# ScanNet/ScanNet

Measured on AMD Instinct MI355X. Metric: RGB-D frames/sec integrated (640x480, 4 mm voxel), higher is better.
Workload: dtype f32; 1 GPU; configs[1]: scene0000_00-scale synthetic stream (5578-frame box-room walk, 640x480 u16 depth, 4 mm voxels, 2^19 hash buckets x 10, 2^20 SDF blocks), frames 5..24 per rank, depth AND colour (a 640x480 RGB8 frame per depth frame, 921 600 B) resident in HBM; frames_per_pass=32, blocks_live_end=34141, alloc_failures=0

## Files before the change

include/scanfuse_internal.h:

```cpp
#ifndef SCANFUSE_INTERNAL_H
#define SCANFUSE_INTERNAL_H

#include "scanfuse.h"

#ifdef __cplusplus
extern "C" {
#endif

int sf_fuser_tune(sf_fuser* f, const char* key, int value);

int sf_fuser_alloc_probe_count(sf_fuser* f, uint64_t* out);

int sf_fuser_alloc_direct_count(sf_fuser* f, uint64_t* out);

int sf_fuser_mc_timing(const sf_fuser* f, double* out, int n);

int sf_zlib_inflate_gpu(const void* src, uint64_t src_bytes, uint64_t expect_bytes, int device, void* dst);
int sf_zlib_inflate_gpu_bench(const void* const* srcs, const uint64_t* src_bytes, int count, uint64_t expect_bytes, int device, int repeats, int skip, double* us_tokens, double* us_copy);

int sf_fuse_run_device_counts(uint64_t out[4]);

int sf_jpeg_decode_gpu_huffman(const uint8_t* data, uint64_t bytes, uint32_t width, uint32_t height, int device, uint8_t* dst_rgb);

int sf_fuser_profile_enable(sf_fuser* f, int on);
// ... 53 lines not shown
```

scannet_amd/csrc/fuser.hip:

```cpp
#include <hip/hip_runtime.h>

#include <algorithm>
#include <climits>
#include <cmath>
#include <cstdlib>
#include <cstring>
#include <string>
#include <vector>

#include "fuser_internal.h"

hipError_t sf_quiesce(sf_fuser* f) {
  hipError_t e = hipSuccess;
  if (f->front) e = hipStreamSynchronize(f->front);
  if (f->front_lo) { const hipError_t e1 = hipStreamSynchronize(f->front_lo); if (e == hipSuccess) e = e1; }
  const hipError_t e2 = hipStreamSynchronize(f->stream);
  return e != hipSuccess ? e : e2;
}

namespace {

bool frame_setup(const sf_params& p, const float* pose, FrameK& f) {
  if (pose[0] == -INFINITY) return false;
  for (int i = 0; i < 12; i++) f.T[i] = pose[i];
// ... 67 lines not shown
  hipStream_t sa = sf_input_stream(f, n, col, sign);
  if (f->overlap && sa != s) {
    if (f->last_front != nullptr && f->last_front != sa) {
      (void)hipEventRecord(f->ev_front_switch, f->last_front);
      (void)hipStreamWaitEvent(sa, f->ev_front_switch, 0);
    }
    f->last_front = sa;
    if (f->serial_tail) {
      (void)hipEventRecord(f->ev_input, s);
      (void)hipStreamWaitEvent(sa, f->ev_input, 0);
      f->serial_tail = false;
    }
    (void)hipStreamWaitEvent(sa, f->ev_fused[sl], 0);
  }
  const bool fuse_pre = f->alloc_ray && n == 1 && sign > 0 && !col && f->pk.inW == 0 && !rs;
  if (!fuse_pre) sf_launch_prepass(f, sl, rs ? n_planes : n, in, sa);
  if (sign > 0) sf_launch_alloc(f, sl, n, bf, in, sa, fuse_pre);
  sf_launch_compact(f, sl, bf, sa);
  if (f->overlap && sa != s) {
    (void)hipEventRecord(f->ev_compact[sl], sa);
    (void)hipStreamWaitEvent(s, f->ev_compact[sl], 0);
  }
  hipEvent_t e0 = nullptr, e1 = nullptr;
  if (f->profile) {
    if (f->events_used == f->events.size()) {
      hipEvent_t a, b;
      if (hipEventCreate(&a) != hipSuccess || hipEventCreate(&b) != hipSuccess) return sf::fail(SF_ERR_DEVICE, "hipEventCreate failed");
      f->events.emplace_back(a, b);
    }
    e0 = f->events[f->events_used].first;
    e1 = f->events[f->events_used].second;
    f->events_used++;
    (void)hipEventRecord(e0, s);
  }
  if (rs) sf_launch_reintegrate(f, sl, col, bt, *rs, s);
  else sf_launch_integrate(f, sl, n, sign, col, bt, s);
  if (f->profile) (void)hipEventRecord(e1, s);
  if (f->overlap && sa != s) (void)hipEventRecord(f->ev_fused[sl], s);
  if (f->overlap && sa == s) f->serial_tail = true;
  f->pipe_beside = f->pipe_overlap == 1 || (f->pipe_overlap < 0 && sf_big_pass(f));
  if ((f->pipe_beside || f->front_prio == 0) && f->front_lo == nullptr && f->overlap) {
    int prio_lo = 0, prio_hi = 0;
    hipError_t e_ = hipSuccess;
    if (f->front_lo_lowest) {
      e_ = hipDeviceGetStreamPriorityRange(&prio_lo, &prio_hi);
      if (e_ == hipSuccess) e_ = hipStreamCreateWithPriority(&f->front_lo, hipStreamNonBlocking, prio_lo);
    } else {
      e_ = hipStreamCreateWithFlags(&f->front_lo, hipStreamNonBlocking);
    }
    if (e_ != hipSuccess) {
// ... 106 lines not shown
    hipError_t e_ = hipMalloc((void**)&(ptr), (bytes));                                           \
    if (e_ != hipSuccess) {                                                                       \
      sf_fuser_destroy(f);                                                                        \
      return sf::fail(SF_ERR_DEVICE, "hipMalloc(%zu bytes) failed: %s", (size_t)(bytes), hipGetErrorString(e_)); \
    }                                                                                             \
  } while (0)
  SF_CREATE_CHECK(hipStreamCreateWithFlags(&f->stream, hipStreamNonBlocking));
  {
    int prio_lo = 0, prio_hi = 0;
    SF_CREATE_CHECK(hipDeviceGetStreamPriorityRange(&prio_lo, &prio_hi));
    SF_CREATE_CHECK(hipStreamCreateWithPriority(&f->front, hipStreamNonBlocking, prio_hi));
    SF_CREATE_CHECK(hipEventCreateWithFlags(&f->ev_front_switch, hipEventDisableTiming));
  }
  for (int q = 0; q < 2; q++) {
    SF_CREATE_CHECK(hipEventCreateWithFlags(&f->ev_compact[q], hipEventDisableTiming));
    SF_CREATE_CHECK(hipEventCreateWithFlags(&f->ev_fused[q], hipEventDisableTiming));
  }
  SF_CREATE_CHECK(hipEventCreateWithFlags(&f->ev_input, hipEventDisableTiming));
  SF_ALLOC(f->table, (size_t)k.total_slots * sizeof(HashEntry));
  {
    uint32_t lines = 1024;
    while ((uint64_t)lines * 64ull < (uint64_t)k.num_blocks && lines < (1u << 24)) lines <<= 1;
    f->brick_lines = lines;
    SF_ALLOC(f->bricks, (size_t)lines * 8 * 16);
  }
  SF_ALLOC(f->heap, (size_t)k.num_blocks * 4);
  SF_ALLOC(f->block_keys, (size_t)k.num_blocks * 8);
  SF_ALLOC(f->block_entry, (size_t)k.num_blocks * 4);
  SF_ALLOC(f->block_flags, (size_t)k.num_blocks);
  SF_ALLOC(f->voxels, (size_t)k.num_blocks * 4096);
// ... 34 lines not shown
#undef SF_CREATE_CHECK
  *out = f;
  return SF_OK;
}

SF_API void sf_fuser_destroy(sf_fuser* f) {
  if (!f) return;
  (void)hipSetDevice(f->device);
  if (f->front) (void)hipStreamSynchronize(f->front);
  if (f->front_lo) (void)hipStreamSynchronize(f->front_lo);
  if (f->stream) (void)hipStreamSynchronize(f->stream);
  for (auto& e : f->events) { (void)hipEventDestroy(e.first); (void)hipEventDestroy(e.second); }
  (void)hipFree(f->table); (void)hipFree(f->bricks); (void)hipFree(f->heap); (void)hipFree(f->block_keys); (void)hipFree(f->block_entry); (void)hipFree(f->block_flags); (void)hipFree(f->voxels);
  for (int q = 0; q < 2; q++) { (void)hipFree(f->depthf2[q]); (void)hipFree(f->color2[q]); (void)hipFree(f->compact2[q]); (void)hipFree(f->cmask2[q]); }
  (void)hipFree(f->counters); (void)hipFree(f->ray_kx); (void)hipFree(f->ray_ky); (void)hipFree(f->void_depth);
  for (int q = 0; q < 2; q++) { if (f->ev_compact[q]) (void)hipEventDestroy(f->ev_compact[q]); if (f->ev_fused[q]) (void)hipEventDestroy(f->ev_fused[q]); }
  if (f->ev_input) (void)hipEventDestroy(f->ev_input);
  if (f->front) { (void)hipStreamSynchronize(f->front); (void)hipStreamDestroy(f->front); }
  if (f->front_lo) { (void)hipStreamSynchronize(f->front_lo); (void)hipStreamDestroy(f->front_lo); }
  if (f->ev_front_switch) (void)hipEventDestroy(f->ev_front_switch);
  for (hipEvent_t e : f->ev_raycast) if (e) (void)hipEventDestroy(e);
  sf_track_release(f);
  sf_align_release(f);
  for (int q = 0; q < sf_fuser::HOST_RING; q++) {
    (void)hipFree(f->staging_depth[q]); (void)hipFree(f->staging_rgb[q]);
    if (f->pinned_depth[q]) (void)hipHostFree(f->pinned_depth[q]);
    if (f->pinned_rgb[q]) (void)hipHostFree(f->pinned_rgb[q]);
    if (f->ev_h2d[q]) (void)hipEventDestroy(f->ev_h2d[q]);
    if (f->ev_consumed[q]) (void)hipEventDestroy(f->ev_consumed[q]);
  }
  if (f->host_mirror) (void)hipHostFree(f->host_mirror);
// ... 70 lines not shown
  return fuse_host(f, depth, rgb, pose, +1);
}
SF_API int sf_fuser_deintegrate(sf_fuser* f, const uint16_t* depth, const uint8_t* rgb, const float pose[16]) {
  return fuse_host(f, depth, rgb, pose, -1);
}
SF_API int sf_fuser_integrate_device(sf_fuser* f, const void* d_depth, const void* d_rgb, const float pose[16]) {
  if (!f || !d_depth || !pose) return sf::fail(SF_ERR_INVALID_ARG, "NULL argument");
  SF_HIP_CHECK(hipSetDevice(f->device));
  return run_frame(f, d_depth, d_rgb, pose, +1);
}
SF_API int sf_fuser_deintegrate_device(sf_fuser* f, const void* d_depth, const void* d_rgb, const float pose[16]) {
  if (!f || !d_depth || !pose) return sf::fail(SF_ERR_INVALID_ARG, "NULL argument");
  SF_HIP_CHECK(hipSetDevice(f->device));
  return run_frame(f, d_depth, d_rgb, pose, -1);
}
static int integrate_batch_device(sf_fuser* f, const void* d_depth, uint64_t frame_stride_bytes, const void* d_rgb, uint64_t rgb_stride_bytes, const float* poses,
                                  uint64_t n) {
  if (!f || !d_depth || !poses) return sf::fail(SF_ERR_INVALID_ARG, "NULL argument");
  SF_HIP_CHECK(hipSetDevice(f->device));
  const void* dd[MAX_BATCH];
  const void* dr[MAX_BATCH];
  const float* pp[MAX_BATCH];
  int m = 0;
  int pass = 0;
  for (uint64_t i = 0; i <= n; i++) {
    if (i < n) {
      if (poses[16 * i] == -INFINITY) { f->frames_skipped++; continue; }
      dd[m] = (const uint8_t*)d_depth + i * frame_stride_bytes;
      dr[m] = d_rgb ? (const uint8_t*)d_rgb + i * rgb_stride_bytes : nullptr;
      pp[m] = poses + 16 * i;
      m++;
    }
    constexpr int ramp = 8;
    int want = f->batch;
    if (ramp < f->batch && n > (uint64_t)ramp) {
      if (n <= (uint64_t)f->batch) want = (int)((n + 1) / 2);
      else if (pass == 0) want = ramp;
      else if (pass < 6) want = std::min(f->batch, ramp << pass);
    }
    if (m == want || (i == n && m > 0)) {
      f->tail_pass = i == n;
      f->head_pass = pass == 0 && n > (uint64_t)m;
      const int rc = run_batch(f, dd, d_rgb ? dr : nullptr, pp, m, +1);
      f->tail_pass = false;
      f->head_pass = false;
      if (rc != SF_OK) return rc;
      m = 0;
      pass++;
    }
  }
  return SF_OK;
}
SF_API int sf_fuser_integrate_batch_device(sf_fuser* f, const void* d_depth, uint64_t frame_stride_bytes, const float* poses, uint64_t n) {
  return integrate_batch_device(f, d_depth, frame_stride_bytes, nullptr, 0, poses, n);
}
SF_API int sf_fuser_integrate_batch_device_rgb(sf_fuser* f, const void* d_depth, uint64_t frame_stride_bytes, const void* d_rgb, uint64_t rgb_stride_bytes,
                                               const float* poses, uint64_t n) {
  if (!d_rgb) return sf::fail(SF_ERR_INVALID_ARG, "NULL colour frames (sf_fuser_integrate_batch_device is the geometry-only entry point)");
  return integrate_batch_device(f, d_depth, frame_stride_bytes, d_rgb, rgb_stride_bytes, poses, n);
}
// ... 122 lines not shown
  if (!f || !key) return sf::fail(SF_ERR_INVALID_ARG, "NULL argument");
  SF_HIP_CHECK(hipSetDevice(f->device));
  SF_HIP_CHECK(sf_quiesce(f));
  const std::string k(key);
  auto in = [&](int lo, int hi) { return value >= lo && value <= hi; };
  if (k == "batch" && in(1, MAX_BATCH)) f->batch = value;
  else if (k == "overlap" && in(0, 1)) f->overlap = value != 0;
  else if (k == "xcd_walk" && in(0, 1)) f->xcd_walk = value != 0;
  else if (k == "pipe" && in(0, 1)) f->pipe_mode = value;
  else if (k == "pipe_overlap" && in(-1, 1)) { f->pipe_overlap = value; f->pipe_beside = value == 1; }
  else if (k == "alloc_group" && in(1, MAX_BATCH)) f->alloc_group = value;
  else if (k == "front_prio" && in(-1, 1)) f->front_prio = value;
  else if (k == "front_lo_lowest" && in(0, 1)) f->front_lo_lowest = value != 0;
  else if (k == "alloc_ray" && in(0, 1)) f->alloc_ray = value != 0;
  else if (k == "tail_wide" && in(0, 1)) f->tail_wide = value;
  else if (k == "brick_cache" && in(0, 1)) {
    f->brick_on = value != 0;
    SF_HIP_CHECK(hipMemsetAsync(f->bricks, 0, (size_t)f->brick_lines * 128, f->stream));
    SF_HIP_CHECK(sf_quiesce(f));
  }
  else return sf::fail(SF_ERR_INVALID_ARG, "sf_fuser_tune: unknown key or value out of range: %s = %d", key, value);
  return SF_OK;
}

int sf_fuser_run_batch(sf_fuser* f, const void* const* d_depth, const void* const* d_rgb, const float* const* poses, int n) {
  if (n < 1 || n > f->batch) return sf::fail(SF_ERR_INVALID_ARG, "batch of %d frames (limit %d)", n, f->batch);
  return run_batch(f, d_depth, d_rgb, poses, n, +1);
}

int sf_fuser_run_batch_ycc(sf_fuser* f, const void* const* d_depth, const void* const* d_planes, const void* const* d_layout, const float* const* poses, int n) {
// ... 92 lines not shown
```

scannet_amd/csrc/fuser_alloc.hip:

```cpp
#include <hip/hip_runtime.h>

#include <algorithm>
#include <climits>
#include <cmath>

#include "fuser_device.h"
#include "fuser_internal.h"

namespace {

__device__ inline int world_to_block(float w, float voxel, float rv) {
  const float q = div_rn(w, voxel, rv);
  const int vi = (int)(q >= 0.0f ? q + 0.5f : q - 0.5f);
  return vi >> 3;
}

constexpr int ALLOC_SET = 256;
constexpr int ALLOC_LIST = 512;
constexpr int ALLOC_SET_PROBES = 32;

template <int WIN_LOG2, bool MULTI>
__global__ __launch_bounds__(256) void k_alloc(const float* __restrict__ depthf_all, HashEntry* table, int32_t* heap,
                                               uint64_t* block_keys, int32_t* block_entry, uint8_t* block_flags, int32_t* counters, ParamsK P,
                                               BatchFrames B, int group_frames, BrickCache bricks) {
// ... 692 lines not shown
  hipLaunchKernelGGL((k_alloc_ray<MULTI>), grid, dim3(256), 0, s, f->depthf2[sl], f->table, f->heap, f->block_keys, f->block_entry, f->block_flags,
                     f->counters, f->pk, bf, gf, raw_depth, f->depthf2[sl], sf_compact_counter(sl));
}

}

void sf_alloc_choose_window(sf_fuser* f, const sf_params* p) {
  const float seg = 2.0f * (p->trunc_base + p->trunc_scale * p->max_integration_dist) / (8.0f * p->voxel_size);
  f->alloc_win64 = seg > 20.0f;
  const float bsz = 8.0f * p->voxel_size;
  const float half_tile = 8.0f * p->max_integration_dist / std::min(p->fx, p->fy);
  const float reach = (p->max_integration_dist + p->trunc_base + p->trunc_scale * p->max_integration_dist) * 1.25f;
  f->alloc_ray = half_tile / bsz <= 4.0f && reach / bsz <= (float)(RW_DEPTH - 6);
}

void sf_launch_alloc(const sf_fuser* f, int sl, int n, const BatchFrames& bf, const BatchIn& in, hipStream_t s, bool fuse_pre) {
  const int group = f->head_pass ? std::min(f->alloc_group, 4) : f->alloc_group;
  const bool win64 = f->alloc_win64 && !f->alloc_ray;
  const int gf = win64 ? 1 : std::min(group, n);
  const dim3 ag((f->p.depth_width + 15) / 16, (f->p.depth_height + 15) / 16, (n + gf - 1) / gf);
  if (f->alloc_ray) {
    const uint16_t* raw_depth = fuse_pre ? in.depth[0] : nullptr;
    if (gf == 1) launch_alloc_ray<false>(f, sl, ag, bf, gf, raw_depth, s);
    else launch_alloc_ray<true>(f, sl, ag, bf, gf, raw_depth, s);
  }
  else if (win64) launch_alloc<6, false>(f, sl, ag, bf, gf, s);
  else if (gf == 1) launch_alloc<5, false>(f, sl, ag, bf, gf, s);
  else launch_alloc<5, true>(f, sl, ag, bf, gf, s);
}
```

scannet_amd/csrc/fuser_compact.hip:

```cpp
#include <hip/hip_runtime.h>

#include <cstring>

#include "fuser_device.h"
#include "fuser_internal.h"

namespace {

constexpr int COMPACT_FEW = 4;

struct CompactArgs {
  const uint64_t* block_keys;
  const int32_t* block_entry;
  const uint8_t* block_flags;
  const HashEntry* table;
  int32_t* compact;
  uint32_t* cmask;
  int32_t* counters;
  int counter_id, all_live;
  ParamsK P;
  BatchFrames B;
};
constexpr int FRAMEK_WORDS = (int)(sizeof(FrameK) / 4);

constexpr int COMPACT_THREADS = 256;
constexpr int COMPACT_WAVES = COMPACT_THREADS / 64;

__global__ __launch_bounds__(COMPACT_THREADS) void k_compactify(CompactArgs A) {
  const uint64_t* __restrict__ block_keys = A.block_keys;
  const int32_t* __restrict__ block_entry = A.block_entry;
  const uint8_t* __restrict__ block_flags = A.block_flags;
  const HashEntry* __restrict__ table = A.table;
  int32_t* __restrict__ compact = A.compact;
  uint32_t* __restrict__ cmask = A.cmask;
// ... 17 lines not shown
    typedef __attribute__((address_space(4))) const uint32_t* karg_t;
    typedef __attribute__((address_space(4))) const char* kbyte_t;
    const karg_t kp = (karg_t)((kbyte_t)__builtin_amdgcn_kernarg_segment_ptr() + offsetof(CompactArgs, B) + offsetof(BatchFrames, f));
    for (int i = threadIdx.x; i < B.n * FRAMEK_WORDS; i += COMPACT_THREADS) s_fk[i] = kp[i];
    __syncthreads();
    uint32_t* fw = reinterpret_cast<uint32_t*>(&F);
    const uint32_t* mine = s_fk + (q < B.n ? q : 0) * FRAMEK_WORDS;
#pragma unroll
    for (int i = 0; i < FRAMEK_WORDS; i++) fw[i] = mine[i];
  }
  for (int base = blockIdx.x * COMPACT_THREADS; base < hw; base += gridDim.x * COMPACT_THREADS) {
    const int i = base + (int)threadIdx.x;
    uint32_t m = 0u;
    if (wide) {
      int4 c = make_int4(0, 0, 0, 0);
      if (i < hw) {
        const uint64_t k = block_keys[i];
        if (k != KEY_EMPTY && !(block_flags[i] & 1)) {
          unpack_key(k, c.x, c.y, c.z);
          c.w = 1;
        }
      }
      s_c[threadIdx.x] = c;
      __syncthreads();
      const uint64_t gmask = fshift == 5 ? 0xFFFFFFFFull : ((1ull << (1 << fshift)) - 1ull);
#pragma unroll 2
      for (int e0 = wave * 64; e0 < wave * 64 + 64; e0 += epi) {
        const int4 cc = s_c[e0 + sub];
        const bool in = cc.w != 0 && q < B.n && block_in_frustum(P, F, cc.x, cc.y, cc.z);
        const uint64_t bal = __ballot(in);
        if (q == 0) s_m[e0 + sub] = (uint32_t)((bal >> (sub << fshift)) & gmask);
      }
      __syncthreads();
      m = s_m[threadIdx.x];
      if (m != 0u) {
        const uint32_t birth = table[block_entry[i]].birth;
        if (birth > B.seq0) {
          const uint32_t d = birth - B.seq0;
          m = d >= 32u ? 0u : (m & ~((1u << d) - 1u));
        }
      }
    }
    const uint64_t bal = __ballot(m != 0u);
    const int rank = __popcll((unsigned long long)(bal & ((1ull << lane) - 1ull)));
    const int wtotal = __popcll((unsigned long long)bal);
    const int wlast = __popcll((unsigned long long)__ballot((m & last_bit) != 0u));
    int pop = __popc(m);
    for (int o = 32; o > 0; o >>= 1) pop += __shfl_xor(pop, o);
    if (lane == 0) { s_wtot[wave] = wtotal; s_wlast[wave] = wlast; s_wpop[wave] = pop; }
    __syncthreads();
    if (threadIdx.x == 0) {
      int total = 0, tlast = 0;
      for (int w = 0; w < COMPACT_WAVES; w++) { total += s_wtot[w]; tlast += s_wlast[w]; }
      s_base = 0;
      if (total) {
        const unsigned long long add = (unsigned long long)(uint32_t)total | ((unsigned long long)(uint32_t)tlast << 32);
        s_base = (int)(uint32_t)atomicAdd(reinterpret_cast<unsigned long long*>(&counters[counter_id]), add);
      }
    } else if (threadIdx.x == 64 && !all_live) {
      int total = 0, tpop = 0;
      for (int w = 0; w < COMPACT_WAVES; w++) { total += s_wtot[w]; tpop += s_wpop[w]; }
      if (total) {
        atomicAdd(reinterpret_cast<unsigned long long*>(&counters[C_TOTAL_LO]), (unsigned long long)tpop);
        atomicAdd(reinterpret_cast<unsigned long long*>(&counters[C_TILES_LO]), (unsigned long long)total);
      }
    }
    __syncthreads();
    int off = s_base;
    for (int w = 0; w < wave; w++) off += s_wtot[w];
    if (m != 0u) {
      compact[off + rank] = i;
      cmask[off + rank] = m;
    }
    __syncthreads();
  }
}

__global__ __launch_bounds__(COMPACT_THREADS) void k_compactify_few(CompactArgs A) {
  const uint64_t* __restrict__ block_keys = A.block_keys;
  const int32_t* __restrict__ block_entry = A.block_entry;
// ... 20 lines not shown
#pragma unroll
    for (int u = 0; u < EU; u++) {
      const int i = base + u * COMPACT_THREADS + (int)threadIdx.x;
      k[u] = i < hw ? block_keys[i] : KEY_EMPTY;
      fl[u] = i < hw ? block_flags[i] : (uint8_t)0;
    }
    int wlast = 0, pop = 0;
#pragma unroll
    for (int u = 0; u < EU; u++) {
      m[u] = 0u;
      if (k[u] != KEY_EMPTY && !(all_live != 1 && (fl[u] & 1))) {
        if (all_live) m[u] = 1u;
        else {
          int bx, by, bz;
          unpack_key(k[u], bx, by, bz);
          for (int qq = 0; qq < B.n; qq++)
            if (block_in_frustum(P, B.f[qq], bx, by, bz)) m[u] |= 1u << qq;
          if (m[u] != 0u && B.n > 1) {
            const uint32_t birth = table[block_entry[base + u * COMPACT_THREADS + (int)threadIdx.x]].birth;
            if (birth > B.seq0) {
              const uint32_t d = birth - B.seq0;
              m[u] = d >= 32u ? 0u : (m[u] & ~((1u << d) - 1u));
            }
          }
        }
      }
      const uint64_t bal = __ballot(m[u] != 0u);
      rank[u] = __popcll((unsigned long long)(bal & ((1ull << lane) - 1ull)));
      if (lane == 0) s_ut[u][wave] = __popcll((unsigned long long)bal);
      wlast += __popcll((unsigned long long)__ballot((m[u] & last_bit) != 0u));
      pop += __popc(m[u]);
    }
    for (int o = 32; o > 0; o >>= 1) pop += __shfl_xor(pop, o);
    if (lane == 0) { s_wlast[wave] = wlast; s_wpop[wave] = pop; }
// ... 7 lines not shown
      s_base = 0;
      if (total) {
        const unsigned long long add = (unsigned long long)(uint32_t)total | ((unsigned long long)(uint32_t)tlast << 32);
        s_base = (int)(uint32_t)atomicAdd(reinterpret_cast<unsigned long long*>(&counters[counter_id]), add);
      }
    } else if (threadIdx.x == 64 && !all_live) {
      int total = 0, tpop = 0;
      for (int w = 0; w < COMPACT_WAVES; w++) {
        tpop += s_wpop[w];
        for (int u = 0; u < EU; u++) total += s_ut[u][w];
      }
      if (total) {
        atomicAdd(reinterpret_cast<unsigned long long*>(&counters[C_TOTAL_LO]), (unsigned long long)tpop);
        atomicAdd(reinterpret_cast<unsigned long long*>(&counters[C_TILES_LO]), (unsigned long long)total);
      }
    }
    __syncthreads();
    int off = s_base;
#pragma unroll
    for (int u = 0; u < EU; u++) {
      int mine = off;
      for (int w = 0; w < COMPACT_WAVES; w++) {
        const int t = s_ut[u][w];
        if (w < wave) mine += t;
        off += t;
      }
      if (m[u] != 0u) {
        compact[mine + rank[u]] = base + u * COMPACT_THREADS + (int)threadIdx.x;
        cmask[mine + rank[u]] = m[u];
      }
    }
    __syncthreads();
  }
}

}

void sf_launch_compact(const sf_fuser* f, int sl, const BatchFrames& bf, hipStream_t s) {
  const CompactArgs a{f->block_keys, f->block_entry, f->block_flags, f->table, f->compact2[sl], f->cmask2[sl], f->counters, sf_compact_counter(sl), 0, f->pk, bf};
  if (bf.n > COMPACT_FEW) hipLaunchKernelGGL(k_compactify, dim3(f->compact_grid * (1024 / COMPACT_THREADS)), dim3(COMPACT_THREADS), 0, s, a);
  else hipLaunchKernelGGL(k_compactify_few, dim3(f->compact_grid * (1024 / COMPACT_THREADS)), dim3(COMPACT_THREADS), 0, s, a);
}

int sf_compact_live(sf_fuser* f, int32_t* n_out, int include_ghosts) {
  SF_HIP_CHECK(sf_quiesce(f));
  BatchFrames dummy;
  std::memset(&dummy, 0, sizeof(dummy));
  dummy.n = 1;
  SF_HIP_CHECK(hipMemsetAsync(&f->counters[C_EXPORT], 0, 8, f->stream));
  hipLaunchKernelGGL(k_compactify_few, dim3(f->compact_grid * (1024 / COMPACT_THREADS)), dim3(COMPACT_THREADS), 0, f->stream, (CompactArgs{f->block_keys, f->block_entry, f->block_flags, f->table, f->compact,
                     f->cmask2[0], f->counters, (int)C_EXPORT, include_ghosts ? 1 : 2, f->pk, dummy}));
  SF_HIP_CHECK(hipMemcpyAsync(n_out, &f->counters[C_EXPORT], 4, hipMemcpyDeviceToHost, f->stream));
  SF_HIP_CHECK(sf_quiesce(f));
  return SF_OK;
}
```

scannet_amd/csrc/fuser_integrate.hip:

```cpp
#include <hip/hip_runtime.h>

#include "fuser_device.h"
#include "fuser_fuse.h"
#include "fuser_internal.h"

namespace {


constexpr int INT_WAVES = 5;
constexpr int INT_NJ = 4;
template <int SIGN, int COLOR, bool TAB, int WM, bool ROWS, int NJ = INT_NJ, bool XR = false>
__global__ __launch_bounds__(256, NJ == 2 ? (XR ? 7 : 8) : INT_WAVES) void k_integrate(uint4* __restrict__ voxels, const uint64_t* __restrict__ block_keys,
                                                   const int32_t* __restrict__ compact, const uint32_t* __restrict__ cmask,
                                                   const float* __restrict__ depthf_all, const uint2* __restrict__ texel_all,
                                                   int32_t* counters, int32_t* host_mirror, int compact_counter, int xcd_walk, ParamsK P,
                                                   BatchTi B) {
  __shared__ float s_rtab[RTAB];
  if (TAB) {
    for (int i = threadIdx.x; i < RTAB; i += 256) s_rtab[i] = 1.0f / (float)(i > 0 ? i : 1);
    __syncthreads();
  }
  const int n = counters[compact_counter];
  const int lane = threadIdx.x & 63;
  const int wave = threadIdx.x >> 6;
  if (blockIdx.x == 0 && threadIdx.x == 0) {
    atomicExch(&counters[C_LAST_BLOCKS], counters[compact_counter + 1]);
    if (host_mirror) *host_mirror = n;
  }
  const int lx = XR ? 0 : (2 * lane) & 7;
  const int ly = XR ? lane & 7 : (lane >> 2) & 7;
  const int lzb = XR ? lane >> 3 : lane >> 5;
  const size_t npx = (size_t)P.W * P.H;
  const int wg_total = (n + 3) >> 2;
  const int chunk = xcd_walk ? (wg_total + 7) >> 3 : wg_total;
  const int lanes = xcd_walk ? 8 : 1;
  const int sub = xcd_walk ? (int)(blockIdx.x & 7) : 0;
  const int per_sub = max(1, (int)gridDim.x / lanes);
  for (int loc = xcd_walk ? (int)(blockIdx.x >> 3) : (int)blockIdx.x; loc < chunk; loc += per_sub) {
    const int i = ((sub * chunk + loc) << 2) + wave;
    if (i >= n) continue;
    const int slot = compact[i];
    uint32_t frames = (uint32_t)__builtin_amdgcn_readfirstlane((int)cmask[i]);
    int bx, by, bz;
    unpack_key(block_keys[slot], bx, by, bz);
    uint4* vb = voxels + (size_t)slot * 256;
    uint4 v[4];
#pragma unroll
    for (int j = 0; j < 4; j++) v[j] = vb[XR ? lane * 4 + j : j * 64 + lane];
    const v2f wx = {(float)(8 * bx + lx) * P.voxel, (float)(8 * bx + lx + 1) * P.voxel};
    const float wy = (float)(8 * by + ly) * P.voxel;
    float wz[4];
    v2f wxp[4];
#pragma unroll
    for (int j = 0; j < 4; j++) {
      wz[j] = (float)(8 * bz + (XR ? 0 : 2 * j) + lzb) * P.voxel;
      wxp[j] = v2f{(float)(8 * bx + 2 * j) * P.voxel, (float)(8 * bx + 2 * j + 1) * P.voxel};
    }
// ... 233 lines not shown
}

bool recip_table_ok(const sf_fuser* f) { return f->p.weight_sample >= 1 && f->p.weight_sample <= RTAB - 256 && f->p.weight_mode == 0; }

int list_grid(const sf_fuser* f, int entries) {
  int grid = (entries + entries / 4 + 4096 + 3) / 4;
  if (grid > f->num_cus * 64) grid = f->num_cus * 64;
  return (grid + 7) & ~7;
}

struct IntegrateLaunch {
  const sf_fuser* f;
  int sl, n;
  const BatchTi& bt;
  hipStream_t s;

  template <int SIGN, int COLOR, bool TAB, int WM, bool ROWS, int NJ = INT_NJ, bool XR = false>
  void integrate() const {
    const int grid = list_grid(f, *f->host_mirror);
    hipLaunchKernelGGL((k_integrate<SIGN, COLOR, TAB, WM, ROWS, NJ, XR>), dim3(grid), dim3(256), 0, s, f->voxels, f->block_keys, f->compact2[sl],
                       f->cmask2[sl], f->depthf2[sl], f->color2[sl], f->counters, f->host_mirror, sf_compact_counter(sl), f->xcd_walk ? 1 : 0, f->pk, bt);
  }
  template <int SIGN, int COLOR, bool TAB, int WM>
  void rows() const {
    if (SIGN < 0 || n == 1) integrate<SIGN, COLOR, TAB, WM, true>();
    else integrate<1, COLOR, TAB, WM, false>();
  }
  template <int SIGN, bool TAB, int WM>
  void colour(bool col) const {
    if (col) rows<SIGN, 1, TAB, WM>();
    else rows<SIGN, 0, TAB, WM>();
  }
  template <int COLOR>
  void xrow(bool wide) const {
    if (wide) integrate<1, COLOR, true, 2, false, 2, true>();
    else integrate<1, COLOR, true, 2, false, INT_NJ, true>();
// ... 14 lines not shown
                     f->xcd_walk ? 1 : 0, read_only, contiguous, sink);
}
template <bool NT>
void launch_tile_rmw_g(const sf_fuser* f, int sl, int G, int grid, int read_only, int contiguous, uint32_t* sink) {
  if (G == 1) launch_tile_rmw<NT, 1>(f, sl, grid, read_only, contiguous, sink);
  else if (G == 2) launch_tile_rmw<NT, 2>(f, sl, grid, read_only, contiguous, sink);
  else launch_tile_rmw<NT, 4>(f, sl, grid, read_only, contiguous, sink);
}

}

int sf_list_grid(const sf_fuser* f, int entries) { return list_grid(f, entries); }

bool sf_pipe_batch(const sf_fuser* f, int n, bool color, int sign) { return sign > 0 && n == 1 && !color && recip_table_ok(f) && f->pipe_mode != 0; }

void sf_launch_integrate(const sf_fuser* f, int sl, int n, int sign, bool col, const BatchTi& bt, hipStream_t s) {
  const IntegrateLaunch L{f, sl, n, bt, s};
  const bool ws1 = f->p.weight_sample == 1 && f->p.weight_mode == 0;
  const bool shipped = ws1 && f->pk.wmax == 255;
  if (sf_pipe_batch(f, n, col, sign)) {
    const bool nt = sf_big_pass(f);
    if (shipped) L.pipe<2>(nt);
    else if (ws1) L.pipe<1>(nt);
    else L.pipe<0>(nt);
  } else if (sign > 0) {
    if (shipped) {
      const int cl = col ? (f->p.colour_first ? 1 : 2) : 0;
      const bool wide = f->tail_pass && f->tail_wide;
      if (cl == 1) L.rows<1, 1, true, 2>();
      else if (n == 1) { if (cl == 2) L.integrate<1, 2, true, 2, true>(); else L.integrate<1, 0, true, 2, true>(); }
      else if (cl == 2) L.xrow<2>(wide);
      else L.xrow<0>(wide);
// ... 48 lines not shown
```

scannet_amd/csrc/fuser_internal.h:

```cpp
#pragma once
#include <hip/hip_runtime.h>

#include <utility>
#include <vector>

#include "common.h"

constexpr uint64_t KEY_EMPTY = ~0ull;
constexpr uint64_t KEY_TOMB = ~0ull - 1ull;
constexpr int MAX_DDA_ITERS = 1024;
constexpr int MAX_PROBES = 4096;
constexpr int MAX_BATCH = 32;
constexpr int DEFAULT_BATCH = 32;

struct HashEntry {
  uint64_t key;
  int32_t ptr;
  uint32_t birth;
};
static_assert(sizeof(HashEntry) == 16, "hash entry is 16 bytes");

struct ParamsK {
  int W, H;
  float fx, fy, mx, my;
// ... 63 lines not shown
enum Counter {
  C_HEAP_FREE = 0,
  C_HIGH_WATER = 2,
  C_ALLOC_FAIL = 3,
  C_SLOTS_USED = 4,
  C_LAST_BLOCKS = 5,
  C_GC_FREED = 7,
  C_IMPORTED = 8,
  C_COMPACT = 16,
  C_COMPACT_B = 18,
  C_EXPORT = 20,
  C_TOTAL_LO = 32,
  C_TILES_LO = 34,
  C_ALLOC_DIRECT = 40,
  C_ALLOC_PROBED = 41,
  C_COUNT = 48
};

__host__ __device__ inline uint64_t pack_key(int x, int y, int z) {
  return (((uint64_t)x & 0x1FFFFFull) << 42) | (((uint64_t)y & 0x1FFFFFull) << 21) | ((uint64_t)z & 0x1FFFFFull);
}
__host__ __device__ inline void unpack_key(uint64_t k, int& x, int& y, int& z) {
  x = ((int)((k >> 42) & 0x1FFFFF) << 11) >> 11;
  y = ((int)((k >> 21) & 0x1FFFFF) << 11) >> 11;
  z = ((int)(k & 0x1FFFFF) << 11) >> 11;
}

__device__ inline uint32_t hash_bucket(int x, int y, int z, uint32_t num_buckets) {
  const uint32_t h = ((uint32_t)x * 73856093u) ^ ((uint32_t)y * 19349669u) ^ ((uint32_t)z * 83492791u);
  return h % num_buckets;
}
__device__ inline uint32_t hash_home(const ParamsK& P, int x, int y, int z) { return hash_bucket(x, y, z, P.num_buckets) * P.bucket_size; }
// ... 92 lines not shown

struct sf_fuser {
  sf_params p;
  ParamsK pk;
  int in_W = 0, in_H = 0;
  size_t in_px = 0;
  int device = 0;
  hipStream_t stream = nullptr;
  hipStream_t front = nullptr;
  hipStream_t front_lo = nullptr;
  hipStream_t last_front = nullptr;
  hipEvent_t ev_front_switch = nullptr;
  int front_prio = -1;
  bool front_lo_lowest = true;
  hipEvent_t ev_compact[2] = {nullptr, nullptr};
  hipEvent_t ev_fused[2] = {nullptr, nullptr};
  hipEvent_t ev_input = nullptr;
  int slot = 0;
  bool serial_tail = false;
  bool overlap = true;
  float* depthf2[2] = {nullptr, nullptr};
  bool head_pass = false;
  bool tail_pass = false;
  int tail_wide = 1;
  uint2* color2[2] = {nullptr, nullptr};
  int32_t* compact2[2] = {nullptr, nullptr};
  uint32_t* cmask2[2] = {nullptr, nullptr};
  int32_t* block_entry = nullptr;
  uint8_t* block_flags = nullptr;
  uint32_t frame_seq = 1;
// ... 14 lines not shown
  void* staging_rgb[HOST_RING] = {nullptr, nullptr, nullptr};
  void* pinned_depth[HOST_RING] = {nullptr, nullptr, nullptr};
  void* pinned_rgb[HOST_RING] = {nullptr, nullptr, nullptr};
  hipEvent_t ev_h2d[HOST_RING] = {nullptr, nullptr, nullptr};
  hipEvent_t ev_consumed[HOST_RING] = {nullptr, nullptr, nullptr};
  int host_slot = 0;
  uint64_t host_frames = 0;
  int32_t* host_mirror = nullptr;
  int num_cus = 256;
  bool alloc_win64 = false;
  bool alloc_ray = false;
  bool xcd_walk = true;
  int pipe_mode = 1;
  bool pipe_beside = false;
  int pipe_overlap = -1;
  int alloc_group = 16;
  int compact_grid = 1024;
  uint64_t frames_integrated = 0, frames_skipped = 0;
  void* void_depth = nullptr;
  int reint_passes = 0;
  bool profile = false;
  void* mc_bounce[2] = {nullptr, nullptr};
  hipEvent_t mc_bounce_ev[2] = {nullptr, nullptr};
  double mc_timing[12] = {0};
  hipEvent_t ev_raycast[3] = {nullptr, nullptr, nullptr};
  struct TrackWork* track = nullptr;
  struct AlignWork* align = nullptr;
  std::vector<std::pair<hipEvent_t, hipEvent_t>> events;
  size_t events_used = 0;
};


hipError_t sf_quiesce(sf_fuser* f);
void sf_track_release(sf_fuser* f);
void sf_align_release(sf_fuser* f);
int sf_order_behind_fronts(sf_fuser* f);
int sf_order_fronts_behind(sf_fuser* f);
bool sf_single_stream_batch(const sf_fuser* f, int n, bool color, int sign);
hipStream_t sf_input_stream(const sf_fuser* f, int n, bool color, int sign);
int sf_compact_live(sf_fuser* f, int32_t* n_out, int include_ghosts = 1);

inline int sf_compact_counter(int sl) { return sl ? (int)C_COMPACT_B : (int)C_COMPACT; }
void sf_launch_prepass(const sf_fuser* f, int sl, int n, const BatchIn& in, hipStream_t s);
void sf_launch_alloc(const sf_fuser* f, int sl, int n, const BatchFrames& bf, const BatchIn& in, hipStream_t s, bool fuse_pre);
void sf_launch_compact(const sf_fuser* f, int sl, const BatchFrames& bf, hipStream_t s);
void sf_launch_integrate(const sf_fuser* f, int sl, int n, int sign, bool col, const BatchTi& bt, hipStream_t s);
void sf_launch_reintegrate(const sf_fuser* f, int sl, bool col, const BatchTi& bt, const ReintSlots& rs, hipStream_t s);
int sf_fuser_run_batch(sf_fuser* f, const void* const* d_depth, const void* const* d_rgb, const float* const* poses, int n);
int sf_fuser_run_batch_ycc(sf_fuser* f, const void* const* d_depth, const void* const* d_planes, const void* const* d_layout, const float* const* poses, int n);
int sf_list_grid(const sf_fuser* f, int entries);
inline int sf_fuser_reintegrate_passes(const sf_fuser* f) { return f->reint_passes; }
bool sf_pipe_batch(const sf_fuser* f, int n, bool color, int sign);
bool sf_big_tile_set(uint32_t tiles);
bool sf_big_pass(const sf_fuser* f);
void sf_alloc_choose_window(sf_fuser* f, const sf_params* p);
void sf_launch_ray_tables(const sf_fuser* f);
void sf_launch_init_heap(const sf_fuser* f);
```

scannet_amd/csrc/fuser_prepass.hip:

```cpp
#include <hip/hip_runtime.h>

#include <algorithm>
#include <cmath>

#include "fuser_internal.h"
#include "jpeg_idct.h"

namespace {

struct YccPicture {
  int ncomp, sx[3], sy[3], cw[3], ch[3], bw[3];
  const uint8_t* plane[3];
  __device__ YccPicture(const SfJpegLayout* __restrict__ L, const uint8_t* planes) {
    const int W = L->width, H = L->height;
    ncomp = L->ncomp;
    const uint8_t* q = planes;
    for (int c = 0; c < 3; c++) {
      const int cc = c < ncomp ? c : 0;
      sx[c] = L->hmax > L->h[cc] ? 2 : 1; sy[c] = L->vmax > L->v[cc] ? 2 : 1;
      cw[c] = (W + sx[c] - 1) >> (sx[c] - 1); ch[c] = (H * L->v[cc] + L->vmax - 1) >> (L->vmax - 1);
      bw[c] = L->bw[cc];
      plane[c] = q;
      if (c < ncomp) q += (size_t)L->bw[cc] * L->bh[cc];
    }
// ... 13 lines not shown
    return (uint32_t)o[0] | ((uint32_t)o[1] << 8) | ((uint32_t)o[2] << 16);
  }
};

__global__ __launch_bounds__(256) void k_prepass(BatchIn in, float* __restrict__ depthf_all, uint2* __restrict__ texel_all, int n,
                                                 float shift, float dmin, float dmax, int32_t* counters, int compact_counter, ParamsK P,
                                                 const float* __restrict__ ray_kx, const float* __restrict__ ray_ky) {
  const int j = blockIdx.y;
  const uint16_t* __restrict__ depth = in.depth[j];
  const uint8_t* __restrict__ rgb = in.rgb[j];
  float* __restrict__ depthf = depthf_all + (size_t)j * n;
  uint2* __restrict__ texel = texel_all + (size_t)j * n;
  const int i0 = (blockIdx.x * 256 + threadIdx.x) * 8;
  if (blockIdx.x == 0 && j == 0 && threadIdx.x == 0) {
    atomicExch(reinterpret_cast<unsigned long long*>(&counters[compact_counter]), 0ull);
  }
  const bool ycc = rgb != nullptr && in.lay[j] != nullptr;
  if (i0 >= n && !ycc) return;
  uint16_t u[8];
  if (P.inW > 0) {
    for (int k = 0; k < 8; k++) {
      const int i = i0 + k;
      if (i >= n) { u[k] = 0; continue; }
      const unsigned xi = (unsigned)((float)(i % P.W) * P.rsx + 0.5f), yi = (unsigned)((float)(i / P.W) * P.rsy + 0.5f);
      u[k] = (xi < (unsigned)P.inW && yi < (unsigned)P.inH) ? depth[(size_t)yi * P.inW + xi] : (uint16_t)0;
    }
  } else if (i0 + 8 <= n) {
    const uint4 raw = *reinterpret_cast<const uint4*>(depth + i0);
    u[0] = raw.x & 0xFFFF; u[1] = raw.x >> 16; u[2] = raw.y & 0xFFFF; u[3] = raw.y >> 16;
    u[4] = raw.z & 0xFFFF; u[5] = raw.z >> 16; u[6] = raw.w & 0xFFFF; u[7] = raw.w >> 16;
// ... 91 lines not shown
```

Before: 35190 frames/s.

## Split batch pass into pre-existing and newborn block lists to overlap alloc with integrate

Adds a split-pass mode that compacts the already-allocated blocks (list A) before allocation runs. Integration of list A starts on the main stream while allocation and a second compaction of newborn blocks (list B, filtered by birth sequence) proceed on the input stream. The list-B integrate then waits only on the second compaction. When the whole request fits in one batch, the pass planner now uses a single full-size pass instead of two halves. The aim is to hide allocation latency behind integration, at the cost of an extra compaction launch, another event dependency, and extra birth lookups in the compaction kernels.

Result: slower. 32130 frames/s (-8.7%).

```diff
diff --git a/include/scanfuse_internal.h b/include/scanfuse_internal.h
--- a/include/scanfuse_internal.h
+++ b/include/scanfuse_internal.h
@@ -8,6 +8,8 @@
 #endif
 
 int sf_fuser_tune(sf_fuser* f, const char* key, int value);
+
+int sf_pass_plan(uint64_t n, int batch, int split_pass, int32_t* sizes, uint8_t* split, uint64_t capacity, uint64_t* count);
 
 int sf_fuser_alloc_probe_count(sf_fuser* f, uint64_t* out);
 
diff --git a/scannet_amd/csrc/fuser.hip b/scannet_amd/csrc/fuser.hip
--- a/scannet_amd/csrc/fuser.hip
+++ b/scannet_amd/csrc/fuser.hip
@@ -105,13 +105,17 @@
     (void)hipStreamWaitEvent(sa, f->ev_fused[sl], 0);
   }
   const bool fuse_pre = f->alloc_ray && n == 1 && sign > 0 && !col && f->pk.inW == 0 && !rs;
+  const bool split = f->split_next && f->split_pass != 0 && n >= 2 && sign > 0 && !rs && !d_lay && !fuse_pre && f->overlap && sa != s;
   if (!fuse_pre) sf_launch_prepass(f, sl, rs ? n_planes : n, in, sa);
-  if (sign > 0) sf_launch_alloc(f, sl, n, bf, in, sa, fuse_pre);
-  sf_launch_compact(f, sl, bf, sa);
-  if (f->overlap && sa != s) {
-    (void)hipEventRecord(f->ev_compact[sl], sa);
-    (void)hipStreamWaitEvent(s, f->ev_compact[sl], 0);
-  }
+  if (split) {
+    sf_launch_compact(f, sl, bf, sa, LIST_A);
+    (void)hipEventRecord(f->ev_compact_a[sl], sa);
+    (void)hipStreamWaitEvent(s, f->ev_compact_a[sl], 0);
+  }
+  if (sign > 0) sf_launch_alloc(f, sl, n, bf, in, sa, fuse_pre, split);
+  sf_launch_compact(f, sl, bf, sa, split ? LIST_B : LIST_WHOLE);
+  if (f->overlap && sa != s) (void)hipEventRecord(f->ev_compact[sl], sa);
+  if (f->overlap && sa != s && !split) (void)hipStreamWaitEvent(s, f->ev_compact[sl], 0);
   hipEvent_t e0 = nullptr, e1 = nullptr;
   if (f->profile) {
     if (f->events_used == f->events.size()) {
@@ -125,6 +129,11 @@
     (void)hipEventRecord(e0, s);
   }
   if (rs) sf_launch_reintegrate(f, sl, col, bt, *rs, s);
+  else if (split) {
+    sf_launch_integrate(f, sl, n, sign, col, bt, s, LIST_A);
+    (void)hipStreamWaitEvent(s, f->ev_compact[sl], 0);
+    sf_launch_integrate(f, sl, n, sign, col, bt, s, LIST_B);
+  }
   else sf_launch_integrate(f, sl, n, sign, col, bt, s);
   if (f->profile) (void)hipEventRecord(e1, s);
   if (f->overlap && sa != s) (void)hipEventRecord(f->ev_fused[sl], s);
@@ -261,6 +270,7 @@
   }
   for (int q = 0; q < 2; q++) {
     SF_CREATE_CHECK(hipEventCreateWithFlags(&f->ev_compact[q], hipEventDisableTiming));
+    SF_CREATE_CHECK(hipEventCreateWithFlags(&f->ev_compact_a[q], hipEventDisableTiming));
     SF_CREATE_CHECK(hipEventCreateWithFlags(&f->ev_fused[q], hipEventDisableTiming));
   }
   SF_CREATE_CHECK(hipEventCreateWithFlags(&f->ev_input, hipEventDisableTiming));
@@ -325,7 +335,7 @@
   (void)hipFree(f->table); (void)hipFree(f->bricks); (void)hipFree(f->heap); (void)hipFree(f->block_keys); (void)hipFree(f->block_entry); (void)hipFree(f->block_flags); (void)hipFree(f->voxels);
   for (int q = 0; q < 2; q++) { (void)hipFree(f->depthf2[q]); (void)hipFree(f->color2[q]); (void)hipFree(f->compact2[q]); (void)hipFree(f->cmask2[q]); }
   (void)hipFree(f->counters); (void)hipFree(f->ray_kx); (void)hipFree(f->ray_ky); (void)hipFree(f->void_depth);
-  for (int q = 0; q < 2; q++) { if (f->ev_compact[q]) (void)hipEventDestroy(f->ev_compact[q]); if (f->ev_fused[q]) (void)hipEventDestroy(f->ev_fused[q]); }
+  for (int q = 0; q < 2; q++) { if (f->ev_compact[q]) (void)hipEventDestroy(f->ev_compact[q]); if (f->ev_compact_a[q]) (void)hipEventDestroy(f->ev_compact_a[q]); if (f->ev_fused[q]) (void)hipEventDestroy(f->ev_fused[q]); }
   if (f->ev_input) (void)hipEventDestroy(f->ev_input);
   if (f->front) { (void)hipStreamSynchronize(f->front); (void)hipStreamDestroy(f->front); }
   if (f->front_lo) { (void)hipStreamSynchronize(f->front_lo); (void)hipStreamDestroy(f->front_lo); }
@@ -426,6 +436,39 @@
   SF_HIP_CHECK(hipSetDevice(f->device));
   return run_frame(f, d_depth, d_rgb, pose, -1);
 }
+namespace {
+constexpr int PASS_RAMP = 8;
+}
+
+SF_API int sf_pass_plan(uint64_t n, int batch, int split_pass, int32_t* sizes, uint8_t* split, uint64_t capacity, uint64_t* count) {
+  if (batch < 1 || batch > MAX_BATCH || split_pass < -1 || split_pass > 1 || !count)
+    return sf::fail(SF_ERR_INVALID_ARG, "sf_pass_plan: batch %d, split_pass %d", batch, split_pass);
+  const bool ramped = PASS_RAMP < batch && n > (uint64_t)PASS_RAMP;
+  const bool fits = ramped && n <= (uint64_t)batch;
+  uint64_t k = 0, left = n;
+  while (left > 0) {
+    int want = batch;
+    if (fits) want = split_pass < 0 ? (int)n : (int)((n + 1) / 2);
+    else if (ramped && k == 0) want = PASS_RAMP;
+    else if (ramped && k < 6) want = std::min(batch, PASS_RAMP << k);
+    const int m = (int)std::min<uint64_t>((uint64_t)want, left);
+    const bool sp = split_pass == 1 || (split_pass < 0 && fits);
+    if (k < capacity) {
+      if (sizes) sizes[k] = m;
+      if (split) split[k] = sp && m >= 2 ? 1 : 0;
+    }
+    left -= (uint64_t)m;
+    k++;
+    if (k >= capacity && k >= 6) {
+      k += (left + (uint64_t)batch - 1) / (uint64_t)batch;
+      left = 0;
+    }
+  }
+  *count = k;
+  if (k > capacity) return sf::fail(SF_ERR_BOUNDS, "sf_pass_plan: %llu passes, room for %llu", (unsigned long long)k, (unsigned long long)capacity);
+  return SF_OK;
+}
+
 static int integrate_batch_device(sf_fuser* f, const void* d_depth, uint64_t frame_stride_bytes, const void* d_rgb, uint64_t rgb_stride_bytes, const float* poses,
                                   uint64_t n) {
   if (!f || !d_depth || !poses) return sf::fail(SF_ERR_INVALID_ARG, "NULL argument");
@@ -433,6 +476,13 @@
   const void* dd[MAX_BATCH];
   const void* dr[MAX_BATCH];
   const float* pp[MAX_BATCH];
+  constexpr int PLANNED = 8;
+  int32_t sizes[PLANNED];
+  uint8_t splits[PLANNED];
+  uint64_t planned = 0;
+  const int rp = sf_pass_plan(n, f->batch, f->split_pass, sizes, splits, PLANNED, &planned);
+  if (rp != SF_OK && rp != SF_ERR_BOUNDS) return rp;
+  if (rp == SF_ERR_BOUNDS) sf::last_error_ref().clear();
   int m = 0;
   int pass = 0;
   for (uint64_t i = 0; i <= n; i++) {
@@ -443,19 +493,15 @@
       pp[m] = poses + 16 * i;
       m++;
     }
-    constexpr int ramp = 8;
-    int want = f->batch;
-    if (ramp < f->batch && n > (uint64_t)ramp) {
-      if (n <= (uint64_t)f->batch) want = (int)((n + 1) / 2);
-      else if (pass == 0) want = ramp;
-      else if (pass < 6) want = std::min(f->batch, ramp << pass);
-    }
+    const int want = pass < PLANNED && (uint64_t)pass < planned ? sizes[pass] : f->batch;
     if (m == want || (i == n && m > 0)) {
       f->tail_pass = i == n;
       f->head_pass = pass == 0 && n > (uint64_t)m;
+      f->split_next = pass < PLANNED && (uint64_t)pass < planned ? splits[pass] != 0 : f->split_pass == 1;
       const int rc = run_batch(f, dd, d_rgb ? dr : nullptr, pp, m, +1);
       f->tail_pass = false;
       f->head_pass = false;
+      f->split_next = false;
       if (rc != SF_OK) return rc;
       m = 0;
       pass++;
@@ -608,6 +654,7 @@
   else if (k == "front_lo_lowest" && in(0, 1)) f->front_lo_lowest = value != 0;
   else if (k == "alloc_ray" && in(0, 1)) f->alloc_ray = value != 0;
   else if (k == "tail_wide" && in(0, 1)) f->tail_wide = value;
+  else if (k == "split_pass" && in(-1, 1)) f->split_pass = value;
   else if (k == "brick_cache" && in(0, 1)) {
     f->brick_on = value != 0;
     SF_HIP_CHECK(hipMemsetAsync(f->bricks, 0, (size_t)f->brick_lines * 128, f->stream));
diff --git a/scannet_amd/csrc/fuser_alloc.hip b/scannet_amd/csrc/fuser_alloc.hip
--- a/scannet_amd/csrc/fuser_alloc.hip
+++ b/scannet_amd/csrc/fuser_alloc.hip
@@ -730,8 +730,8 @@
   f->alloc_ray = half_tile / bsz <= 4.0f && reach / bsz <= (float)(RW_DEPTH - 6);
 }
 
-void sf_launch_alloc(const sf_fuser* f, int sl, int n, const BatchFrames& bf, const BatchIn& in, hipStream_t s, bool fuse_pre) {
-  const int group = f->head_pass ? std::min(f->alloc_group, 4) : f->alloc_group;
+void sf_launch_alloc(const sf_fuser* f, int sl, int n, const BatchFrames& bf, const BatchIn& in, hipStream_t s, bool fuse_pre, bool beside_integrate) {
+  const int group = f->head_pass && !beside_integrate ? std::min(f->alloc_group, 4) : f->alloc_group;
   const bool win64 = f->alloc_win64 && !f->alloc_ray;
   const int gf = win64 ? 1 : std::min(group, n);
   const dim3 ag((f->p.depth_width + 15) / 16, (f->p.depth_height + 15) / 16, (n + gf - 1) / gf);
diff --git a/scannet_amd/csrc/fuser_compact.hip b/scannet_amd/csrc/fuser_compact.hip
--- a/scannet_amd/csrc/fuser_compact.hip
+++ b/scannet_amd/csrc/fuser_compact.hip
@@ -18,6 +18,8 @@
   uint32_t* cmask;
   int32_t* counters;
   int counter_id, all_live;
+  int mirror_id;
+  uint32_t born_from;
   ParamsK P;
   BatchFrames B;
 };
@@ -65,27 +67,34 @@
     uint32_t m = 0u;
     if (wide) {
       int4 c = make_int4(0, 0, 0, 0);
+      uint32_t born = 0u;
       if (i < hw) {
         const uint64_t k = block_keys[i];
         if (k != KEY_EMPTY && !(block_flags[i] & 1)) {
-          unpack_key(k, c.x, c.y, c.z);
-          c.w = 1;
+          if (A.born_from != 0u) born = table[block_entry[i]].birth;
+          if (born >= A.born_from) {
+            unpack_key(k, c.x, c.y, c.z);
+            c.w = 1;
+          }
         }
       }
       s_c[threadIdx.x] = c;
+      s_m[threadIdx.x] = 0u;
       __syncthreads();
       const uint64_t gmask = fshift == 5 ? 0xFFFFFFFFull : ((1ull << (1 << fshift)) - 1ull);
+      if (A.born_from == 0u || __ballot(c.w != 0) != 0ull) {
 #pragma unroll 2
-      for (int e0 = wave * 64; e0 < wave * 64 + 64; e0 += epi) {
-        const int4 cc = s_c[e0 + sub];
-        const bool in = cc.w != 0 && q < B.n && block_in_frustum(P, F, cc.x, cc.y, cc.z);
-        const uint64_t bal = __ballot(in);
-        if (q == 0) s_m[e0 + sub] = (uint32_t)((bal >> (sub << fshift)) & gmask);
+        for (int e0 = wave * 64; e0 < wave * 64 + 64; e0 += epi) {
+          const int4 cc = s_c[e0 + sub];
+          const bool in = cc.w != 0 && q < B.n && block_in_frustum(P, F, cc.x, cc.y, cc.z);
+          const uint64_t bal = __ballot(in);
+          if (q == 0) s_m[e0 + sub] = (uint32_t)((bal >> (sub << fshift)) & gmask);
+        }
       }
       __syncthreads();
       m = s_m[threadIdx.x];
       if (m != 0u) {
-        const uint32_t birth = table[block_entry[i]].birth;
+        const uint32_t birth = A.born_from != 0u ? born : table[block_entry[i]].birth;
         if (birth > B.seq0) {
           const uint32_t d = birth - B.seq0;
           m = d >= 32u ? 0u : (m & ~((1u << d) - 1u));
@@ -115,6 +124,11 @@
         atomicAdd(reinterpret_cast<unsigned long long*>(&counters[C_TOTAL_LO]), (unsigned long long)tpop);
         atomicAdd(reinterpret_cast<unsigned long long*>(&counters[C_TILES_LO]), (unsigned long long)total);
       }
+    }
+    else if (threadIdx.x == 128 && A.mirror_id >= 0) {
+      int total = 0, tlast = 0;
+      for (int w = 0; w < COMPACT_WAVES; w++) { total += s_wtot[w]; tlast += s_wlast[w]; }
+      if (total) atomicAdd(reinterpret_cast<unsigned long long*>(&counters[A.mirror_id]), (unsigned long long)(uint32_t)total | ((unsigned long long)(uint32_t)tlast << 32));
     }
     __syncthreads();
     int off = s_base;
@@ -165,10 +179,12 @@
         else {
           int bx, by, bz;
           unpack_key(k[u], bx, by, bz);
-          for (int qq = 0; qq < B.n; qq++)
-            if (block_in_frustum(P, B.f[qq], bx, by, bz)) m[u] |= 1u << qq;
+          const uint32_t born = A.born_from != 0u ? table[block_entry[base + u * COMPACT_THREADS + (int)threadIdx.x]].birth : 0u;
+          if (born >= A.born_from)
+            for (int qq = 0; qq < B.n; qq++)
+              if (block_in_frustum(P, B.f[qq], bx, by, bz)) m[u] |= 1u << qq;
           if (m[u] != 0u && B.n > 1) {
-            const uint32_t birth = table[block_entry[base + u * COMPACT_THREADS + (int)threadIdx.x]].birth;
+            const uint32_t birth = A.born_from != 0u ? born : table[block_entry[base + u * COMPACT_THREADS + (int)threadIdx.x]].birth;
             if (birth > B.seq0) {
               const uint32_t d = birth - B.seq0;
               m[u] = d >= 32u ? 0u : (m[u] & ~((1u << d) - 1u));
@@ -206,6 +222,13 @@
         atomicAdd(reinterpret_cast<unsigned long long*>(&counters[C_TOTAL_LO]), (unsigned long long)tpop);
         atomicAdd(reinterpret_cast<unsigned long long*>(&counters[C_TILES_LO]), (unsigned long long)total);
       }
+    } else if (threadIdx.x == 128 && A.mirror_id >= 0) {
+      int total = 0, tlast = 0;
+      for (int w = 0; w < COMPACT_WAVES; w++) {
+        tlast += s_wlast[w];
+        for (int u = 0; u < EU; u++) total += s_ut[u][w];
+      }
+      if (total) atomicAdd(reinterpret_cast<unsigned long long*>(&counters[A.mirror_id]), (unsigned long long)(uint32_t)total | ((unsigned long long)(uint32_t)tlast << 32));
     }
     __syncthreads();
     int off = s_base;
@@ -228,8 +251,9 @@
 
 }
 
-void sf_launch_compact(const sf_fuser* f, int sl, const BatchFrames& bf, hipStream_t s) {
-  const CompactArgs a{f->block_keys, f->block_entry, f->block_flags, f->table, f->compact2[sl], f->cmask2[sl], f->counters, sf_compact_counter(sl), 0, f->pk, bf};
+void sf_launch_compact(const sf_fuser* f, int sl, const BatchFrames& bf, hipStream_t s, ListPart part) {
+  const CompactArgs a{f->block_keys, f->block_entry, f->block_flags, f->table, f->compact2[sl], f->cmask2[sl], f->counters, sf_compact_counter(sl), 0,
+                      part == LIST_A ? sf_split_counter(sl) : -1, part == LIST_B ? bf.seq0 : 0u, f->pk, bf};
   if (bf.n > COMPACT_FEW) hipLaunchKernelGGL(k_compactify, dim3(f->compact_grid * (1024 / COMPACT_THREADS)), dim3(COMPACT_THREADS), 0, s, a);
   else hipLaunchKernelGGL(k_compactify_few, dim3(f->compact_grid * (1024 / COMPACT_THREADS)), dim3(COMPACT_THREADS), 0, s, a);
 }
@@ -241,7 +265,7 @@
   dummy.n = 1;
   SF_HIP_CHECK(hipMemsetAsync(&f->counters[C_EXPORT], 0, 8, f->stream));
   hipLaunchKernelGGL(k_compactify_few, dim3(f->compact_grid * (1024 / COMPACT_THREADS)), dim3(COMPACT_THREADS), 0, f->stream, (CompactArgs{f->block_keys, f->block_entry, f->block_flags, f->table, f->compact,
-                     f->cmask2[0], f->counters, (int)C_EXPORT, include_ghosts ? 1 : 2, f->pk, dummy}));
+                     f->cmask2[0], f->counters, (int)C_EXPORT, include_ghosts ? 1 : 2, -1, 0u, f->pk, dummy}));
   SF_HIP_CHECK(hipMemcpyAsync(n_out, &f->counters[C_EXPORT], 4, hipMemcpyDeviceToHost, f->stream));
   SF_HIP_CHECK(sf_quiesce(f));
   return SF_OK;
diff --git a/scannet_amd/csrc/fuser_integrate.hip b/scannet_amd/csrc/fuser_integrate.hip
--- a/scannet_amd/csrc/fuser_integrate.hip
+++ b/scannet_amd/csrc/fuser_integrate.hip
@@ -13,19 +13,21 @@
 __global__ __launch_bounds__(256, NJ == 2 ? (XR ? 7 : 8) : INT_WAVES) void k_integrate(uint4* __restrict__ voxels, const uint64_t* __restrict__ block_keys,
                                                    const int32_t* __restrict__ compact, const uint32_t* __restrict__ cmask,
                                                    const float* __restrict__ depthf_all, const uint2* __restrict__ texel_all,
-                                                   int32_t* counters, int32_t* host_mirror, int compact_counter, int xcd_walk, ParamsK P,
-                                                   BatchTi B) {
+                                                   int32_t* counters, int32_t* host_mirror, int compact_counter, int begin_counter, int xcd_walk,
+                                                   ParamsK P, BatchTi B) {
   __shared__ float s_rtab[RTAB];
   if (TAB) {
     for (int i = threadIdx.x; i < RTAB; i += 256) s_rtab[i] = 1.0f / (float)(i > 0 ? i : 1);
     __syncthreads();
   }
-  const int n = counters[compact_counter];
+  const int end = counters[compact_counter];
+  const int begin = begin_counter >= 0 ? counters[begin_counter] : 0;
+  const int n = end - begin;
   const int lane = threadIdx.x & 63;
   const int wave = threadIdx.x >> 6;
-  if (blockIdx.x == 0 && threadIdx.x == 0) {
+  if (blockIdx.x == 0 && threadIdx.x == 0 && host_mirror) {
     atomicExch(&counters[C_LAST_BLOCKS], counters[compact_counter + 1]);
-    if (host_mirror) *host_mirror = n;
+    *host_mirror = end;
   }
   const int lx = XR ? 0 : (2 * lane) & 7;
   const int ly = XR ? lane & 7 : (lane >> 2) & 7;
@@ -39,8 +41,8 @@
   for (int loc = xcd_walk ? (int)(blockIdx.x >> 3) : (int)blockIdx.x; loc < chunk; loc += per_sub) {
     const int i = ((sub * chunk + loc) << 2) + wave;
     if (i >= n) continue;
-    const int slot = compact[i];
-    uint32_t frames = (uint32_t)__builtin_amdgcn_readfirstlane((int)cmask[i]);
+    const int slot = compact[begin + i];
+    uint32_t frames = (uint32_t)__builtin_amdgcn_readfirstlane((int)cmask[begin + i]);
     int bx, by, bz;
     unpack_key(block_keys[slot], bx, by, bz);
     uint4* vb = voxels + (size_t)slot * 256;
@@ -304,12 +306,14 @@
   int sl, n;
   const BatchTi& bt;
   hipStream_t s;
+  ListPart part;
 
   template <int SIGN, int COLOR, bool TAB, int WM, bool ROWS, int NJ = INT_NJ, bool XR = false>
   void integrate() const {
-    const int grid = list_grid(f, *f->host_mirror);
+    const int grid = list_grid(f, part == LIST_B ? 0 : *f->host_mirror);
     hipLaunchKernelGGL((k_integrate<SIGN, COLOR, TAB, WM, ROWS, NJ, XR>), dim3(grid), dim3(256), 0, s, f->voxels, f->block_keys, f->compact2[sl],
-                       f->cmask2[sl], f->depthf2[sl], f->color2[sl], f->counters, f->host_mirror, sf_compact_counter(sl), f->xcd_walk ? 1 : 0, f->pk, bt);
+                       f->cmask2[sl], f->depthf2[sl], f->color2[sl], f->counters, part == LIST_A ? nullptr : f->host_mirror,
+                       part == LIST_A ? sf_split_counter(sl) : sf_compact_counter(sl), part == LIST_B ? sf_split_counter(sl) : -1, f->xcd_walk ? 1 : 0, f->pk, bt);
   }
   template <int SIGN, int COLOR, bool TAB, int WM>
   void rows() const {
@@ -354,8 +358,8 @@
 
 bool sf_pipe_batch(const sf_fuser* f, int n, bool color, int sign) { return sign > 0 && n == 1 && !color && recip_table_ok(f) && f->pipe_mode != 0; }
 
-void sf_launch_integrate(const sf_fuser* f, int sl, int n, int sign, bool col, const BatchTi& bt, hipStream_t s) {
-  const IntegrateLaunch L{f, sl, n, bt, s};
+void sf_launch_integrate(const sf_fuser* f, int sl, int n, int sign, bool col, const BatchTi& bt, hipStream_t s, ListPart part) {
+  const IntegrateLaunch L{f, sl, n, bt, s, part};
   const bool ws1 = f->p.weight_sample == 1 && f->p.weight_mode == 0;
   const bool shipped = ws1 && f->pk.wmax == 255;
   if (sf_pipe_batch(f, n, col, sign)) {
diff --git a/scannet_amd/csrc/fuser_internal.h b/scannet_amd/csrc/fuser_internal.h
--- a/scannet_amd/csrc/fuser_internal.h
+++ b/scannet_amd/csrc/fuser_internal.h
@@ -101,8 +101,12 @@
   C_TILES_LO = 34,
   C_ALLOC_DIRECT = 40,
   C_ALLOC_PROBED = 41,
-  C_COUNT = 48
-};
+  C_SPLIT = 64,
+  C_SPLIT_B = 66,
+  C_COUNT = 96
+};
+constexpr int C_SPLIT_OFF = C_SPLIT - C_COMPACT;
+static_assert(C_SPLIT_B - C_COMPACT_B == C_SPLIT_OFF, "a slot's list-A counter sits C_SPLIT_OFF words behind its list counter (k_prepass zeroes both)");
 
 __host__ __device__ inline uint64_t pack_key(int x, int y, int z) {
   return (((uint64_t)x & 0x1FFFFFull) << 42) | (((uint64_t)y & 0x1FFFFFull) << 21) | ((uint64_t)z & 0x1FFFFFull);
@@ -225,6 +229,7 @@
   int front_prio = -1;
   bool front_lo_lowest = true;
   hipEvent_t ev_compact[2] = {nullptr, nullptr};
+  hipEvent_t ev_compact_a[2] = {nullptr, nullptr};
   hipEvent_t ev_fused[2] = {nullptr, nullptr};
   hipEvent_t ev_input = nullptr;
   int slot = 0;
@@ -269,6 +274,8 @@
   int pipe_mode = 1;
   bool pipe_beside = false;
   int pipe_overlap = -1;
+  int split_pass = -1;
+  bool split_next = false;
   int alloc_group = 16;
   int compact_grid = 1024;
   uint64_t frames_integrated = 0, frames_skipped = 0;
@@ -296,10 +303,12 @@
 int sf_compact_live(sf_fuser* f, int32_t* n_out, int include_ghosts = 1);
 
 inline int sf_compact_counter(int sl) { return sl ? (int)C_COMPACT_B : (int)C_COMPACT; }
+inline int sf_split_counter(int sl) { return sf_compact_counter(sl) + C_SPLIT_OFF; }
+enum ListPart { LIST_WHOLE = 0, LIST_A = 1, LIST_B = 2 };
 void sf_launch_prepass(const sf_fuser* f, int sl, int n, const BatchIn& in, hipStream_t s);
-void sf_launch_alloc(const sf_fuser* f, int sl, int n, const BatchFrames& bf, const BatchIn& in, hipStream_t s, bool fuse_pre);
-void sf_launch_compact(const sf_fuser* f, int sl, const BatchFrames& bf, hipStream_t s);
-void sf_launch_integrate(const sf_fuser* f, int sl, int n, int sign, bool col, const BatchTi& bt, hipStream_t s);
+void sf_launch_alloc(const sf_fuser* f, int sl, int n, const BatchFrames& bf, const BatchIn& in, hipStream_t s, bool fuse_pre, bool beside_integrate = false);
+void sf_launch_compact(const sf_fuser* f, int sl, const BatchFrames& bf, hipStream_t s, ListPart part = LIST_WHOLE);
+void sf_launch_integrate(const sf_fuser* f, int sl, int n, int sign, bool col, const BatchTi& bt, hipStream_t s, ListPart part = LIST_WHOLE);
 void sf_launch_reintegrate(const sf_fuser* f, int sl, bool col, const BatchTi& bt, const ReintSlots& rs, hipStream_t s);
 int sf_fuser_run_batch(sf_fuser* f, const void* const* d_depth, const void* const* d_rgb, const float* const* poses, int n);
 int sf_fuser_run_batch_ycc(sf_fuser* f, const void* const* d_depth, const void* const* d_planes, const void* const* d_layout, const float* const* poses, int n);
diff --git a/scannet_amd/csrc/fuser_prepass.hip b/scannet_amd/csrc/fuser_prepass.hip
--- a/scannet_amd/csrc/fuser_prepass.hip
+++ b/scannet_amd/csrc/fuser_prepass.hip
@@ -51,6 +51,7 @@
   const int i0 = (blockIdx.x * 256 + threadIdx.x) * 8;
   if (blockIdx.x == 0 && j == 0 && threadIdx.x == 0) {
     atomicExch(reinterpret_cast<unsigned long long*>(&counters[compact_counter]), 0ull);
+    atomicExch(reinterpret_cast<unsigned long long*>(&counters[compact_counter + C_SPLIT_OFF]), 0ull);
   }
   const bool ycc = rgb != nullptr && in.lay[j] != nullptr;
   if (i0 >= n && !ycc) return;
```
